# yaramohamadi/Pairwise_Sample_Optimization

Measured on AMD Instinct MI355X. Metric: PSO train-step imgs/sec (paired 1024² SDXL) at 1/2/4/8 MI355X, higher is better.
Workload: dtype bf16; 1 GPU; C2: SDXL-Turbo PSO train step, LoRA r=32 grads, 2 pairs/GPU/micro-step, gas 2, 2-step sampler (T=1); global_batch=4, seq_len=4096, resolution=1024, parallelism=dp1, launch=eager

## Files before the change

pairwise_sample_optimization_amd/csrc/attention.hip:

```cpp
#include "common.h"

#include <type_traits>

#define ATT_D 64
#define ATT_KT 64
#define ATT_THREADS 256

typedef __attribute__((address_space(3))) s16x4 lds_s16x4;

__device__ __forceinline__ int swz_row(int r, int c) { return r * ATT_D + ((c ^ (r & 7)) << 3); }
__device__ __forceinline__ int swz_tr(int r, int c) { return r * ATT_D + ((c ^ (((r >> 1) & 3) << 1)) << 3); }

__device__ __forceinline__ s16x4 tr_read(const bf16_t* img, int r0, int col0, int lane) {
  const int li = lane & 15;
  const int q = li >> 2, p = li & 3;
  const int row = r0 + q;
  const int col = col0 + 4 * p;
  const int off = swz_tr(row, col >> 3) + (col & 7);
  return __builtin_amdgcn_ds_read_tr16_b64_v4i16((lds_s16x4*)(img + off));
}

__device__ __forceinline__ s16x4 tr_read_asm(const bf16_t* img, int r0, int col0, int lane) {
  const int li = lane & 15;
  const int q = li >> 2, p = li & 3;
// ... 380 lines not shown
#pragma unroll
          for (int r = 0; r < 4; ++r)
            if (kbase + kj * 16 + 4 * g + r >= a.Sk) s[qi][kj][r] = -INFINITY;
    }
    float mx[QI];
    bool grow = false;
#pragma unroll
    for (int qi = 0; qi < QI; ++qi) {
      float m = vmax3(s[qi][0][0], s[qi][0][1], s[qi][0][2]);
      m = vmax3(m, s[qi][0][3], s[qi][1][0]);
      m = vmax3(m, s[qi][1][1], s[qi][1][2]);
      m = vmax3(m, s[qi][1][3], s[qi][2][0]);
      m = vmax3(m, s[qi][2][1], s[qi][2][2]);
      m = vmax3(m, s[qi][2][3], s[qi][3][0]);
      m = vmax3(m, s[qi][3][1], s[qi][3][2]);
      m = vmax2(m, s[qi][3][3]);
      mx[qi] = LG ? m : rowmax4_asm(m);
      grow |= mx[qi] > m_run[qi] + thr;
    }
    if (__any(grow)) {
#pragma unroll
      for (int qi = 0; qi < QI; ++qi) {
        const float m_new = fmaxf(m_run[qi], LG ? rowmax4_asm(mx[qi]) : mx[qi]);
        const float alpha = fast_exp2((m_run[qi] - m_new) * c2);
        lsum[qi] *= alpha;
#pragma unroll
        for (int dt = 0; dt < 4; ++dt) o[qi][dt] *= alpha;
        m_run[qi] = m_new;
      }
    }
#pragma unroll
    for (int qi = 0; qi < QI; ++qi) {
      const float mc = m_run[qi] * c2;
#pragma unroll
      for (int kj = 0; kj < 4; ++kj)
#pragma unroll
        for (int r = 0; r < 4; ++r) s[qi][kj][r] = fast_exp2(fmaf(s[qi][kj][r], c2, -mc));
    }
    lds_wait8(vr0);
    s16x4 vr1[8];
#pragma unroll
    for (int dt = 0; dt < 4; ++dt) {
      vr1[2 * dt] = tr_read_imm<VOFF + 2 * 2048>(vbase[dt]);
      vr1[2 * dt + 1] = tr_read_imm<VOFF + 3 * 2048>(vbase[dt]);
    }
#pragma unroll
    for (int ks = 0; ks < 2; ++ks) {
      if (ks == 1) lds_wait8(vr1);
      bf16x8 pf[QI];
#pragma unroll
      for (int qi = 0; qi < QI; ++qi) {
        pf[qi] = pack_p(s[qi][2 * ks], s[qi][2 * ks + 1]);
        lsum[qi] = mfma16x16x32(ones, pf[qi], lsum[qi]);
      }
#pragma unroll
      for (int dt = 0; dt < 4; ++dt) {
        const bf16x8 vf = ks == 0 ? cat_frag(vr0[2 * dt], vr0[2 * dt + 1]) : cat_frag(vr1[2 * dt], vr1[2 * dt + 1]);
#pragma unroll
        for (int qi = 0; qi < QI; ++qi) o[qi][dt] = mfma16x16x32(vf, pf[qi], o[qi][dt]);
      }
    }
  };
  for (int kt = 0; kt < nkt; kt += STG) {
    tile(ic<0>{}, kt);
    if (kt + 1 < nkt) tile(ic<1>{}, kt + 1);
    if (kt + 2 < nkt) tile(ic<2>{}, kt + 2);
  }

  bf16_t* O = a.o + b * a.so_b + h * ATT_D;
#pragma unroll
  for (int qi = 0; qi < QI; ++qi) {
    const float l = lsum[qi][0];
    const int qr = q0 + qi * 16 + c;
    if (qr >= a.Sq) continue;
    const float inv = 1.f / l;
#pragma unroll
    for (int dt = 0; dt < 4; ++dt) {
      const f32x4 v = o[qi][dt];
      *reinterpret_cast<uint2*>(O + (long)qr * a.ldo + dt * 16 + 4 * g) =
          make_uint2(pack2bf(v[0] * inv, v[1] * inv), pack2bf(v[2] * inv, v[3] * inv));
    }
    if (a.lse && g == 0)
      a.lse[((long)b * a.H + h) * a.Sq + qr] = (m_run[qi] * c2 + log2f(l)) * 0.69314718055994531f;
  }
}

template <int KJ, int STG, bool PF = false, bool ONE = false>
__global__ __launch_bounds__(ATT_THREADS, KJ == 2 ? 2 : 1) void attn_bwd_dkv_kernel(AttnArgs a, int nkb) {
  constexpr int IMG = ATT_KT * ATT_D;
  constexpr int NIMG = ONE ? 2 : 4;
  constexpr int PIECES = 2 * NIMG;
  extern __shared__ __attribute__((aligned(16))) bf16_t att_dyn[];
  bf16_t* const sbase = att_dyn;
  float* const sLD = reinterpret_cast<float*>(att_dyn + STG * NIMG * IMG);
  const int tid = threadIdx.x, lane = tid & 63;
  const int wave = __builtin_amdgcn_readfirstlane(tid >> 6);
  const int g = lane >> 4, c = lane & 15;
  const int bid = xcd_remap(blockIdx.x, gridDim.x);
  const int per_bh = nkb * a.q_split;
  const int bh = bid / per_bh, rem = bid - bh * per_bh;
  const int split = rem / nkb, kb = rem - split * nkb;
  const int h = bh % a.H, b = bh / a.H;
  const int k0 = kb * (64 * KJ) + wave * (16 * KJ);

  const bf16_t* Q = a.q + b * a.sq_b + h * ATT_D;
  const bf16_t* K = a.k + b * a.sk_b + h * ATT_D;
  const bf16_t* V = a.v + b * a.sv_b + h * ATT_D;
  const bf16_t* DO = a.dO + b * a.sdo_b + h * ATT_D;
  const float* LSE = a.lse2 + ((long)b * a.H + h) * a.Sq;
  const float* DEL = a.delta + ((long)b * a.H + h) * a.Sq;
  const float c2 = a.scale_log2;

  const int nqt = (a.Sq + ATT_KT - 1) / ATT_KT;
  const int per = (nqt + a.q_split - 1) / a.q_split;
  const int qa = split * per, qb = min(nqt, qa + per);
  const int n = qb > qa ? qb - qa : 0;

  const int prow = lane >> 3, pch = lane & 7;
  const int lcR = pch ^ prow;
  const int lcT = pch ^ (2 * ((prow >> 1) & 3));
  const __amdgpu_buffer_rsrc_t rQ =
      __builtin_amdgcn_make_buffer_rsrc((void*)Q, (short)0, (int)(((long)(a.Sq - 1) * a.ldq + ATT_D) * 2), 0x00020000);
  const __amdgpu_buffer_rsrc_t rO =
      __builtin_amdgcn_make_buffer_rsrc((void*)DO, (short)0, (int)(((long)(a.Sq - 1) * a.lddo + ATT_D) * 2), 0x00020000);
  const __amdgpu_buffer_rsrc_t rL =
      __builtin_amdgcn_make_buffer_rsrc((void*)(wave == 0 ? LSE : DEL), (short)0, a.Sq * 4, 0x00020000);
  unsigned qro[2], qto[2], oro[2], oto[2];
#pragma unroll
  for (int pw = 0; pw < 2; ++pw) {
    const int row = (wave * 2 + pw) * 8 + prow;
    qro[pw] = (unsigned)(row * (int)a.ldq + lcR * 8) * 2u;
    qto[pw] = (unsigned)(row * (int)a.ldq + lcT * 8) * 2u;
    oro[pw] = (unsigned)(row * (int)a.lddo + lcR * 8) * 2u;
    oto[pw] = (unsigned)(row * (int)a.lddo + lcT * 8) * 2u;
  }
  const int qstep = ATT_KT * (int)a.ldq * 2, ostep = ATT_KT * (int)a.lddo * 2;
  auto issue = [&](int qt, int buf) {
    bf16_t* img = sbase + buf * NIMG * IMG;
    if (wave < 2)
      __builtin_amdgcn_raw_ptr_buffer_load_lds(rL, (att_lds_void*)(sLD + (buf * 2 + wave) * 64), 4, lane * 4,
                                               qt * ATT_KT * 4, 0, 0);
#pragma unroll
    for (int pw = 0; pw < 2; ++pw) {
      const int piece = wave * 2 + pw;
      if constexpr (ONE) {
        __builtin_amdgcn_raw_ptr_buffer_load_lds(rQ, (att_lds_void*)(img + piece * 8 * ATT_D), 16, qto[pw], qt * qstep,
                                                 0, 0);
        __builtin_amdgcn_raw_ptr_buffer_load_lds(rO, (att_lds_void*)(img + IMG + piece * 8 * ATT_D), 16, oto[pw],
                                                 qt * ostep, 0, 0);
        continue;
      }
      __builtin_amdgcn_raw_ptr_buffer_load_lds(rQ, (att_lds_void*)(img + piece * 8 * ATT_D), 16, qro[pw], qt * qstep, 0, 0);
      __builtin_amdgcn_raw_ptr_buffer_load_lds(rQ, (att_lds_void*)(img + IMG + piece * 8 * ATT_D), 16, qto[pw], qt * qstep,
                                               0, 0);
      __builtin_amdgcn_raw_ptr_buffer_load_lds(rO, (att_lds_void*)(img + 2 * IMG + piece * 8 * ATT_D), 16, oro[pw],
                                               qt * ostep, 0, 0);
      __builtin_amdgcn_raw_ptr_buffer_load_lds(rO, (att_lds_void*)(img + 3 * IMG + piece * 8 * ATT_D), 16, oto[pw],
                                               qt * ostep, 0, 0);
    }
  };

  bf16x8 kf[KJ][2], vf[KJ][2];
#pragma unroll
  for (int kj = 0; kj < KJ; ++kj) {
    const int kr = min(k0 + kj * 16 + c, a.Sk - 1);
#pragma unroll
// ... 798 lines not shown
#pragma unroll
          for (int r = 0; r < 4; ++r) dsT[qi][kj][r] = fast_exp2(fmaf(sacc[r], a.scale_log2, -lq[qi])) * pacc[r];
        }
      }
    }
    s16x4 kr[2][8];
#pragma unroll
    for (int ks = 0; ks < 2; ++ks)
#pragma unroll
      for (int dt = 0; dt < 4; ++dt) {
        kr[ks][2 * dt] = tr_read_asm(sKt, (2 * ks) * 16 + 4 * g, dt * 16, lane);
        kr[ks][2 * dt + 1] = tr_read_asm(sKt, (2 * ks + 1) * 16 + 4 * g, dt * 16, lane);
      }
    bf16x8 pf[2][2];
#pragma unroll
    for (int ks = 0; ks < 2; ++ks)
#pragma unroll
      for (int qi = 0; qi < 2; ++qi) pf[ks][qi] = pack_p(dsT[qi][2 * ks], dsT[qi][2 * ks + 1]);
    lds_wait8(kr[0]);
    lds_wait8(kr[1]);
#pragma unroll
    for (int ks = 0; ks < 2; ++ks) {
#pragma unroll
      for (int dt = 0; dt < 4; ++dt) {
        const bf16x8 kf = cat_frag(kr[ks][2 * dt], kr[ks][2 * dt + 1]);
#pragma unroll
        for (int qi = 0; qi < 2; ++qi)
          dq[qi][dt] = mfma16x16x32(kf, pf[ks][qi], dq[qi][dt]);
      }
    }
    };
    if (kbase + ATT_KT > a.Sk) body(std::true_type{});
    else body(std::false_type{});
  };
  for (int kt = 0; kt < nkt; kt += STG) {
    tile(ic<0>{}, kt);
    if (kt + 1 < nkt) tile(ic<1>{}, kt + 1);
    if (kt + 2 < nkt) tile(ic<2>{}, kt + 2);
    if constexpr (STG > 3)
      if (kt + 3 < nkt) tile(ic<3>{}, kt + 3);
  }
  const float sc = a.scale_log2 * 0.69314718055994531f;
  bf16_t* DQ = a.dq + b * a.sdq_b + h * ATT_D;
#pragma unroll
  for (int qi = 0; qi < 2; ++qi) {
    const int qr = q0 + qi * 16 + c;
    if (qr >= a.Sq) continue;
#pragma unroll
    for (int dt = 0; dt < 4; ++dt) {
      const f32x4 v = dq[qi][dt];
      *reinterpret_cast<uint2*>(DQ + (long)qr * a.lddq + dt * 16 + 4 * g) =
          make_uint2(pack2bf(v[0] * sc, v[1] * sc), pack2bf(v[2] * sc, v[3] * sc));
    }
  }
}

__global__ void reduce_splits_kernel(long rows, int cols, int nsplit, const float* __restrict__ src_k,
                                     const float* __restrict__ src_v, long split_stride, bf16_t* __restrict__ dst_k,
                                     long ldd_k, bf16_t* __restrict__ dst_v, long ldd_v) {
  const float* __restrict__ src = blockIdx.y ? src_v : src_k;
  bf16_t* __restrict__ dst = blockIdx.y ? dst_v : dst_k;
  const long ldd = blockIdx.y ? ldd_v : ldd_k;
  const int c4 = cols / 4;
  for (long i = blockIdx.x * (long)blockDim.x + threadIdx.x; i < rows * c4; i += (long)gridDim.x * blockDim.x) {
    const long r = i / c4;
    const int cc = (int)(i - r * c4) * 4;
    float4 acc = *reinterpret_cast<const float4*>(src + r * cols + cc);
    for (int sp = 1; sp < nsplit; ++sp) {
      const float4 v = *reinterpret_cast<const float4*>(src + sp * split_stride + r * cols + cc);
      acc.x += v.x; acc.y += v.y; acc.z += v.z; acc.w += v.w;
    }
    *reinterpret_cast<uint2*>(dst + r * ldd + cc) = make_uint2(pack2bf(acc.x, acc.y), pack2bf(acc.z, acc.w));
  }
}

#ifdef PSO_BENCH_KNOBS
static int g_attn_fwd_variant = 0;
static bool g_attn_vsum = false;
static int g_attn_bwd_variant = 0;
static bool g_attn_pp_trace = false;
static int g_attn_xqs = 0;
#else
static constexpr int g_attn_fwd_variant = 0, g_attn_bwd_variant = 0, g_attn_xqs = 0;
#endif

static int cross_qsplit(int B, int H, int Sq, int Sk) {
  if (Sk > 256) return 1;
  if (Sk <= XK_KP && g_attn_bwd_variant != 7) {
    int qs = g_attn_xqs > 0 ? g_attn_xqs : 512 / (H * B);
    const int nqt = cdiv(Sq, ATT_KT);
    if (qs > nqt) qs = nqt;
    return qs < 1 ? 1 : qs;
  }
  const int nqt = cdiv(Sq, ATT_KT);
  int qs = cdiv(512, (long)cdiv(Sk, 128) * H * B);
  if (qs > nqt) qs = nqt;
  return qs < 1 ? 1 : qs;
}


static bool a16(const void* p, long ld) { return (((uintptr_t)p) & 15) == 0 && (ld % 8) == 0; }
static bool a8(const void* p, long ld) { return (((uintptr_t)p) & 7) == 0 && (ld % 4) == 0; }

extern "C" {

#ifdef PSO_BENCH_KNOBS
int pso_attn_pp_trace(unsigned long long* out) {
  return hipMemcpyFromSymbol(out, HIP_SYMBOL(g_pp_trace), sizeof(g_pp_trace)) == hipSuccess ? 0 : 1;
}

void pso_attention_set_variant(int v) {
  g_attn_fwd_variant = v % 10;
  g_attn_bwd_variant = (v / 10) % 10;
  g_attn_vsum = (v / 100) % 10 == 1;
  g_attn_pp_trace = (v / 1000) % 10 == 1;
  g_attn_xqs = (v / 10000) % 100;
}
#endif

int pso_attention_fwd(int B, int H, int Sq, int Sk, const void* q, long ldq, long sq_b, const void* k, long ldk,
                      long sk_b, const void* v, long ldv, long sv_b, float scale, void* o, long ldo, long so_b,
                      float* lse, void* stream) {
  PSO_ARG_CHECK(B > 0 && H > 0 && Sq > 0 && Sk > 0, "pso_attention_fwd: bad shape");
  PSO_ARG_CHECK(q && k && v && o, "pso_attention_fwd: null");
  PSO_ARG_CHECK(a16(q, ldq) && a16(k, ldk) && a16(v, ldv) && (((uintptr_t)o) & 7) == 0 && (ldo % 4) == 0,
                "pso_attention_fwd: operands need 16-B aligned rows");
  AttnArgs a{};
  a.q = (const bf16_t*)q; a.k = (const bf16_t*)k; a.v = (const bf16_t*)v;
  a.ldq = ldq; a.ldk = ldk; a.ldv = ldv; a.sq_b = sq_b; a.sk_b = sk_b; a.sv_b = sv_b;
  a.o = (bf16_t*)o; a.ldo = ldo; a.so_b = so_b; a.lse = lse;
  a.Sq = Sq; a.Sk = Sk; a.H = H; a.scale_log2 = scale * 1.4426950408889634f;
  const int nq4 = cdiv(Sq, 256), nq2 = cdiv(Sq, 128);
  const int fv = g_attn_fwd_variant;
  const int qsel = fv >= 5 ? fv - 5 : fv;
  const bool big = qsel == 4 || ((qsel == 0 || qsel == 1) && (long)nq4 * H * B >= 1024 && Sk > 128);
  hipStream_t st = (hipStream_t)stream;
#ifdef PSO_BENCH_KNOBS
  if (g_attn_vsum) {
    if (big) attn_fwd_kernel<4, false><<<nq4 * H * B, ATT_THREADS, 0, st>>>(a, nq4);
    else attn_fwd_kernel<2, false><<<nq2 * H * B, ATT_THREADS, 0, st>>>(a, nq2);
    return pso_check_launch("pso_attention_fwd");
  } else if (fv >= 5) {
    if (big) attn_fwd_kernel<4><<<nq4 * H * B, ATT_THREADS, 0, st>>>(a, nq4);
    else attn_fwd_kernel<2><<<nq2 * H * B, ATT_THREADS, 0, st>>>(a, nq2);
    return pso_check_launch("pso_attention_fwd");
  } else if (fv == 1) {
    if (big) attn_fwd2_kernel<4, true><<<nq4 * H * B, ATT_THREADS, 0, st>>>(a, nq4);
    else attn_fwd2_kernel<2, true><<<nq2 * H * B, ATT_THREADS, 0, st>>>(a, nq2);
    return pso_check_launch("pso_attention_fwd");
  }
#endif
  if (big) {
    attn_fwd2_kernel<4><<<nq4 * H * B, ATT_THREADS, 0, st>>>(a, nq4);
  } else {
    attn_fwd2_kernel<2><<<nq2 * H * B, ATT_THREADS, 0, st>>>(a, nq2);
  }
  return pso_check_launch("pso_attention_fwd");
}

size_t pso_attention_bwd_ws_bytes(int B, int H, int Sq, int Sk) {
  size_t d = (size_t)B * H * Sq * sizeof(float);
  const int qs = cross_qsplit(B, H, Sq, Sk);
  size_t acc = qs > 1 ? 2 * (size_t)qs * B * Sk * H * ATT_D * sizeof(float) : 0;
  return 2 * (((d + 255) / 256) * 256) + acc;
}

int pso_attention_bwd(int B, int H, int Sq, int Sk, const void* q, long ldq, long sq_b, const void* k, long ldk,
                      long sk_b, const void* v, long ldv, long sv_b, const void* o, long ldo, long so_b,
                      const float* lse, const void* dO, long lddo, long sdo_b, float scale, void* dq, long lddq,
                      long sdq_b, void* dk, long lddk, long sdk_b, void* dv, long lddv, long sdv_b, void* ws,
                      size_t ws_bytes, void* stream) {
  PSO_ARG_CHECK(B > 0 && H > 0 && Sq > 0 && Sk > 0, "pso_attention_bwd: bad shape");
  PSO_ARG_CHECK(q && k && v && o && lse && dO && dq && dk && dv && ws, "pso_attention_bwd: null");
  PSO_ARG_CHECK(ws_bytes >= pso_attention_bwd_ws_bytes(B, H, Sq, Sk), "pso_attention_bwd: workspace too small");
  PSO_ARG_CHECK(a16(q, ldq) && a16(k, ldk) && a16(v, ldv) && a16(o, ldo) && a16(dO, lddo),
                "pso_attention_bwd: operands need 16-B aligned rows");
  PSO_ARG_CHECK(a8(dq, lddq) && a8(dk, lddk) && a8(dv, lddv),
                "pso_attention_bwd: dq/dk/dv need 8-B aligned rows (pointer % 8 == 0, row stride % 4 == 0)");
  PSO_ARG_CHECK(cross_qsplit(B, H, Sq, Sk) == 1 || (sdk_b == (long)Sk * lddk && sdv_b == (long)Sk * lddv),
                "pso_attention_bwd: the query-split path needs dk/dv batch strides of Sk rows "
                "(sdk_b == Sk*lddk, sdv_b == Sk*lddv)");
  hipStream_t st = (hipStream_t)stream;
  AttnArgs a{};
  a.q = (const bf16_t*)q; a.k = (const bf16_t*)k; a.v = (const bf16_t*)v;
  a.ldq = ldq; a.ldk = ldk; a.ldv = ldv; a.sq_b = sq_b; a.sk_b = sk_b; a.sv_b = sv_b;
  a.o = (bf16_t*)o; a.ldo = ldo; a.so_b = so_b; a.lse = (float*)lse;
  a.Sq = Sq; a.Sk = Sk; a.H = H; a.scale_log2 = scale * 1.4426950408889634f;
  a.dO = (const bf16_t*)dO; a.lddo = lddo; a.sdo_b = sdo_b;
  const size_t dsz = (((size_t)B * H * Sq * sizeof(float) + 255) / 256) * 256;
  float* delta = (float*)ws;
  a.delta = delta;
  a.lse2 = (float*)((char*)ws + dsz);
  a.dq = (bf16_t*)dq; a.dk = (bf16_t*)dk; a.dv = (bf16_t*)dv;
  a.lddq = lddq; a.lddk = lddk; a.lddv = lddv; a.sdq_b = sdq_b; a.sdk_b = sdk_b; a.sdv_b = sdv_b;
  const size_t doff = 2 * dsz;
  const int nkb = cdiv(Sk, 128);
  const int qsplit = cross_qsplit(B, H, Sq, Sk);
  const long part = (long)B * Sk * H * ATT_D;
  if (qsplit > 1) {
    a.dk_acc = (float*)((char*)ws + doff);
    a.dv_acc = a.dk_acc + qsplit * part;
  }
  a.q_split = qsplit;
  a.nbatch = B;
  const dim3 gq(cdiv(Sq, 128), H, B);
  const bool xpath = Sk <= XK_KP && g_attn_bwd_variant != 7;
  if (xpath) {
    attn_bwd_x_kernel<<<dim3(qsplit * H * B), ATT_THREADS, 0, st>>>(a);
  } else {
#ifdef PSO_BENCH_KNOBS
  const int bv = g_attn_bwd_variant;
  if (bv == 3 || bv == 1) attn_bwd_dq_kernel<3, false><<<gq, ATT_THREADS, 0, st>>>(a);
  else if (bv == 6) attn_bwd_dq_kernel<4, true><<<gq, ATT_THREADS, 0, st>>>(a);
  else attn_bwd_dq_kernel<3, true><<<gq, ATT_THREADS, 0, st>>>(a);
  const int nkb4 = cdiv(Sk, 256);
  const bool kj4 = g_attn_bwd_variant == 4;
  if (kj4) {
    const size_t shm = 3 * (4 * ATT_KT * ATT_D * sizeof(bf16_t) + 2 * 64 * sizeof(float));
    static bool attr4 = false;
    if (!attr4) {
      (void)hipFuncSetAttribute((const void*)attn_bwd_dkv_kernel<4, 3>, hipFuncAttributeMaxDynamicSharedMemorySize,
                                (int)shm);
      attr4 = true;
    }
    attn_bwd_dkv_kernel<4, 3><<<nkb4 * qsplit * H * B, ATT_THREADS, shm, st>>>(a, nkb4);
  } else if ((bv == 8 || bv == 9) && qsplit == 1) {
    constexpr int PST = 4;
    const size_t shm = PST * (2 * ATT_KT * ATT_D * sizeof(bf16_t) + 2 * 64 * sizeof(float));
    static bool attr8 = false;
    if (!attr8) {
      (void)hipFuncSetAttribute((const void*)attn_bwd_dkv_pp_kernel<PST>, hipFuncAttributeMaxDynamicSharedMemorySize,
                                (int)shm);
      (void)hipFuncSetAttribute((const void*)attn_bwd_dkv_pp_kernel<PST, true>,
                                hipFuncAttributeMaxDynamicSharedMemorySize, (int)shm);
// ... 50 lines not shown
```

pairwise_sample_optimization_amd/csrc/gemm_skinny.hip:

```cpp
#include "common.h"

#include <cstdlib>

__device__ __attribute__((aligned(16))) uint4 g_skinny_zero[4];

namespace {

constexpr int SK_W = 8;

template <int NJ, int SK_MT, int SK_U_ = 0>
__global__ __launch_bounds__(64 * SK_W) void gemm_skinny_nt_kernel(int M, int N, int K, const bf16_t* __restrict__ A,
                                                                   long lda, const bf16_t* __restrict__ W, long ldw,
                                                                   float alpha, void* __restrict__ out, long ldo,
                                                                   int out_f32, int accumulate) {
  constexpr int SK_U = SK_U_ > 0 ? SK_U_ : ((NJ <= 2 && SK_MT <= 2) ? 4 : 2);
  __shared__ f32x4 red[SK_W][NJ][64];
  const int lane = threadIdx.x & 63, wave = threadIdx.x >> 6;
  const int fr = lane & 15, fk = lane >> 4;
  const int r0 = blockIdx.x * (16 * SK_MT);
  const int grp = blockIdx.y;
  A += (long)grp * K;
  W += (long)grp * K;
  const bf16_t* zero = reinterpret_cast<const bf16_t*>(g_skinny_zero);
  const bf16_t* arow[SK_MT];
#pragma unroll
  for (int t = 0; t < SK_MT; ++t) arow[t] = A + (long)min(r0 + t * 16 + fr, M - 1) * lda;
  const bf16_t* wrow[NJ];
  bool wok[NJ];
#pragma unroll
  for (int j = 0; j < NJ; ++j) {
    wok[j] = j * 16 + fr < N;
    wrow[j] = W + (long)min(j * 16 + fr, N - 1) * ldw;
  }
  const int nc = (K + 31) / 32;
  f32x4 acc[SK_MT][NJ];
#pragma unroll
  for (int t = 0; t < SK_MT; ++t)
#pragma unroll
    for (int j = 0; j < NJ; ++j) acc[t][j] = f32x4{0.f, 0.f, 0.f, 0.f};

  for (int c0 = wave; c0 < nc; c0 += SK_W * SK_U) {
    bf16x8 af[SK_U][SK_MT], bfr[SK_U][NJ];
#pragma unroll
    for (int u = 0; u < SK_U; ++u) {
      const int k = (c0 + u * SK_W) * 32 + fk * 8;
      const bool ok = k < K;
#pragma unroll
      for (int t = 0; t < SK_MT; ++t) af[u][t] = *reinterpret_cast<const bf16x8*>(ok ? arow[t] + k : zero);
#pragma unroll
      for (int j = 0; j < NJ; ++j) bfr[u][j] = *reinterpret_cast<const bf16x8*>((ok && wok[j]) ? wrow[j] + k : zero);
    }
    __builtin_amdgcn_sched_barrier(0);
#pragma unroll
    for (int u = 0; u < SK_U; ++u)
#pragma unroll
      for (int t = 0; t < SK_MT; ++t)
#pragma unroll
        for (int j = 0; j < NJ; ++j)
          acc[t][j] = mfma16x16x32(bfr[u][j], af[u][t], acc[t][j]);
  }
#pragma unroll
  for (int t = 0; t < SK_MT; ++t) {
    if (t > 0) __syncthreads();
#pragma unroll
    for (int j = 0; j < NJ; ++j) red[wave][j][lane] = acc[t][j];
    __syncthreads();
    for (int idx = threadIdx.x; idx < NJ * 64; idx += 64 * SK_W) {
      const int l = idx & 63, j = idx >> 6;
      f32x4 s = red[0][j][l];
#pragma unroll
      for (int w = 1; w < SK_W; ++w) s += red[w][j][l];
      const int m = r0 + t * 16 + (l & 15);
      const int n = j * 16 + (l >> 4) * 4;
      if (m >= M || n >= N) continue;
      float v0 = s[0] * alpha, v1 = s[1] * alpha, v2 = s[2] * alpha, v3 = s[3] * alpha;
      const long o = (long)m * ldo + (long)grp * N + n;
      if (out_f32) {
        float4* po = reinterpret_cast<float4*>(reinterpret_cast<float*>(out) + o);
        if (accumulate) {
          const float4 old = *po;
          v0 += old.x; v1 += old.y; v2 += old.z; v3 += old.w;
        }
        *po = make_float4(v0, v1, v2, v3);
      } else {
        *reinterpret_cast<uint2*>(reinterpret_cast<bf16_t*>(out) + o) = make_uint2(pack2bf(v0, v1), pack2bf(v2, v3));
      }
    }
  }
}

#ifdef PSO_BENCH_KNOBS
static int skinny_variant() {
  static int v = -1;
  if (v < 0) {
    const char* e = getenv("PSO_SKINNY_VARIANT");
    v = e ? atoi(e) : 0;
  }
  return v;
}
#else
static constexpr int skinny_variant() { return 0; }
#endif

template <int NJ>
int launch_skinny(int M, int N, int K, const bf16_t* a, long lda, const bf16_t* w, long ldw, float alpha, void* out,
                  long ldo, int out_f32, int accumulate, int groups, hipStream_t st) {
  const int var = NJ <= 2 ? skinny_variant() : 0;
#ifdef PSO_BENCH_KNOBS
  if (var == 1 || var == 3) {
    const dim3 grid((M + 15) / 16, groups);
    if (var == 1) {
      pso_note_kernel("gemm_skinny_nt_kernel<%d, %d, %d>", NJ, 1, 8);
      gemm_skinny_nt_kernel<NJ, 1, 8><<<grid, 64 * SK_W, 0, st>>>(M, N, K, a, lda, w, ldw, alpha, out, ldo, out_f32,
                                                                    accumulate);
    } else {
      pso_note_kernel("gemm_skinny_nt_kernel<%d, %d, %d>", NJ, 1, 4);
      gemm_skinny_nt_kernel<NJ, 1, 4><<<grid, 64 * SK_W, 0, st>>>(M, N, K, a, lda, w, ldw, alpha, out, ldo, out_f32,
                                                                    accumulate);
    }
    return pso_check_launch("pso_gemm(skinny)");
  }
  if (var == 2) {
    const dim3 grid((M + 31) / 32, groups);
    pso_note_kernel("gemm_skinny_nt_kernel<%d, %d, %d>", NJ, 2, 8);
    gemm_skinny_nt_kernel<NJ, 2, 8><<<grid, 64 * SK_W, 0, st>>>(M, N, K, a, lda, w, ldw, alpha, out, ldo, out_f32,
                                                                accumulate);
    return pso_check_launch("pso_gemm(skinny)");
  }
#endif
  const bool k40 = var != 4 && (K + 31) / 32 > SK_W * 4 && (K + 31) / 32 <= SK_W * 5;
  const bool five = NJ <= 6 && k40, five4 = NJ <= 2 && k40;
  constexpr int U5 = NJ <= 6 ? 5 : 4, U5m = NJ <= 6 ? 5 : 0, U5d = NJ <= 2 ? 5 : 0;
  if ((long)((M + 31) / 32) * groups < 128) {
    const dim3 grid((M + 15) / 16, groups);
    if (five) {
      pso_note_kernel("gemm_skinny_nt_kernel<%d, %d, %d>", NJ, 1, U5);
      gemm_skinny_nt_kernel<NJ, 1, U5><<<grid, 64 * SK_W, 0, st>>>(M, N, K, a, lda, w, ldw, alpha, out, ldo, out_f32,
                                                                    accumulate);
    } else {
      pso_note_kernel("gemm_skinny_nt_kernel<%d, %d, %d>", NJ, 1, 4);
      gemm_skinny_nt_kernel<NJ, 1, 4><<<grid, 64 * SK_W, 0, st>>>(M, N, K, a, lda, w, ldw, alpha, out, ldo, out_f32,
                                                                    accumulate);
    }
  } else if ((long)((M + 63) / 64) * groups >= 256) {
    const dim3 grid((M + 63) / 64, groups);
    if (five4) {
      pso_note_kernel("gemm_skinny_nt_kernel<%d, %d, %d>", NJ, 4, U5d);
      gemm_skinny_nt_kernel<NJ, 4, U5d><<<grid, 64 * SK_W, 0, st>>>(M, N, K, a, lda, w, ldw, alpha, out, ldo, out_f32,
                                                                    accumulate);
    } else {
      pso_note_kernel("gemm_skinny_nt_kernel<%d, %d, 0>", NJ, 4);
      gemm_skinny_nt_kernel<NJ, 4><<<grid, 64 * SK_W, 0, st>>>(M, N, K, a, lda, w, ldw, alpha, out, ldo, out_f32,
                                                               accumulate);
    }
  } else {
    const dim3 grid((M + 31) / 32, groups);
    if (five) {
      pso_note_kernel("gemm_skinny_nt_kernel<%d, %d, %d>", NJ, 2, U5m);
      gemm_skinny_nt_kernel<NJ, 2, U5m><<<grid, 64 * SK_W, 0, st>>>(M, N, K, a, lda, w, ldw, alpha, out, ldo, out_f32,
                                                                    accumulate);
    } else {
      pso_note_kernel("gemm_skinny_nt_kernel<%d, %d, 0>", NJ, 2);
      gemm_skinny_nt_kernel<NJ, 2><<<grid, 64 * SK_W, 0, st>>>(M, N, K, a, lda, w, ldw, alpha, out, ldo, out_f32,
                                                               accumulate);
    }
  }
  return pso_check_launch("pso_gemm(skinny)");
}

}

int pso_gemm_skinny_nt(int M, int N, int K, const void* A, long lda, const void* W, long ldw, float alpha, void* out,
                       long ldo, int out_f32, int accumulate, int groups, hipStream_t st) {
  const int nj = (N + 15) / 16;
  auto a = (const bf16_t*)A;
  auto w = (const bf16_t*)W;
  switch (nj) {
    case 1: return launch_skinny<1>(M, N, K, a, lda, w, ldw, alpha, out, ldo, out_f32, accumulate, groups, st);
    case 2: return launch_skinny<2>(M, N, K, a, lda, w, ldw, alpha, out, ldo, out_f32, accumulate, groups, st);
    case 3: case 4: return launch_skinny<4>(M, N, K, a, lda, w, ldw, alpha, out, ldo, out_f32, accumulate, groups, st);
    case 5: case 6: return launch_skinny<6>(M, N, K, a, lda, w, ldw, alpha, out, ldo, out_f32, accumulate, groups, st);
    default: return launch_skinny<8>(M, N, K, a, lda, w, ldw, alpha, out, ldo, out_f32, accumulate, groups, st);
  }
}
```

Before: 37.99 imgs/s.

## Add dedicated cross-attention forward kernel and coalesced row loads in skinny GEMM

Adds attn_fwd_x_kernel for short-key (cross) attention. It keeps the whole K/V (at most two tiles) resident in LDS and loops several query blocks per workgroup, with a q-split grid. Output rows are staged through per-wave LDS so stores are coalesced 16-byte rows. Separately, the skinny GEMM now loads A/W as contiguous row lines and transposes the fragments across lanes with ds_bpermute, trading extra cross-lane permutes for better global-load coalescing. Both paths are on by default, and the old skinny layout is only reachable through a bench knob.

```diff
diff --git a/pairwise_sample_optimization_amd/csrc/attention.hip b/pairwise_sample_optimization_amd/csrc/attention.hip
--- a/pairwise_sample_optimization_amd/csrc/attention.hip
+++ b/pairwise_sample_optimization_amd/csrc/attention.hip
@@ -486,6 +486,242 @@
     }
     if (a.lse && g == 0)
       a.lse[((long)b * a.H + h) * a.Sq + qr] = (m_run[qi] * c2 + log2f(l)) * 0.69314718055994531f;
+  }
+}
+
+__global__ __launch_bounds__(ATT_THREADS, 3) void attn_fwd_x_kernel(AttnArgs a, int nqb, int qsplit) {
+  constexpr int QI = 2;
+  constexpr int OLD = ATT_D + 8;
+  __shared__ __attribute__((aligned(16))) bf16_t sKV[2][2][ATT_KT * ATT_D];
+  __shared__ __attribute__((aligned(16))) bf16_t sO[ATT_THREADS / 64][16 * OLD];
+  const int tid = threadIdx.x, lane = tid & 63;
+  const int wave = __builtin_amdgcn_readfirstlane(tid >> 6);
+  const int g = lane >> 4, c = lane & 15;
+  const int lr = lane >> 2, lc = lane & 3;
+  const int bid = xcd_remap(blockIdx.x, gridDim.x);
+  const int bh = bid / qsplit, split = bid - bh * qsplit;
+  const int h = bh % a.H, b = bh / a.H;
+  const int per = (nqb + qsplit - 1) / qsplit;
+  const int qa = split * per, qe = min(nqb, qa + per);
+  if (qa >= qe) return;
+
+  const bf16_t* Q = a.q + b * a.sq_b + h * ATT_D;
+  const bf16_t* K = a.k + b * a.sk_b + h * ATT_D;
+  const bf16_t* V = a.v + b * a.sv_b + h * ATT_D;
+  bf16_t* O = a.o + b * a.so_b + h * ATT_D;
+  const float c2 = a.scale_log2;
+  const float thr = ATT_RESCALE_LOG2 / c2;
+
+  auto qload = [&](uint4 (&r)[QI][2], int qb) {
+#pragma unroll
+    for (int qi = 0; qi < QI; ++qi) {
+      const int qr = min(qb * (64 * QI) + wave * (16 * QI) + qi * 16 + lr, a.Sq - 1);
+#pragma unroll
+      for (int ds = 0; ds < 2; ++ds)
+        r[qi][ds] = *reinterpret_cast<const uint4*>(Q + (long)qr * a.ldq + ds * 32 + 8 * lc);
+    }
+  };
+  uint4 qraw[QI][2];
+  qload(qraw, qa);
+
+  const int prow = lane >> 3, pch = lane & 7;
+  const int lcK = pch ^ prow;
+  const int lcV = pch ^ (2 * ((prow >> 1) & 3));
+  const int nkt = (a.Sk + ATT_KT - 1) / ATT_KT;
+  const __amdgpu_buffer_rsrc_t rK =
+      __builtin_amdgcn_make_buffer_rsrc((void*)K, (short)0, (int)(((long)(a.Sk - 1) * a.ldk + ATT_D) * 2), 0x00020000);
+  const __amdgpu_buffer_rsrc_t rV =
+      __builtin_amdgcn_make_buffer_rsrc((void*)V, (short)0, (int)(((long)(a.Sk - 1) * a.ldv + ATT_D) * 2), 0x00020000);
+  const int kstep = ATT_KT * (int)a.ldk * 2, vstep = ATT_KT * (int)a.ldv * 2;
+#pragma unroll
+  for (int kt = 0; kt < 2; ++kt) {
+    if (kt < nkt) {
+#pragma unroll
+      for (int pw = 0; pw < 2; ++pw) {
+        const int piece = wave * 2 + pw;
+        const int row = piece * 8 + prow;
+        __builtin_amdgcn_raw_ptr_buffer_load_lds(rK, (att_lds_void*)(sKV[kt][0] + piece * 8 * ATT_D), 16,
+                                                 (unsigned)(row * (int)a.ldk + lcK * 8) * 2u, kt * kstep, 0, 0);
+        __builtin_amdgcn_raw_ptr_buffer_load_lds(rV, (att_lds_void*)(sKV[kt][1] + piece * 8 * ATT_D), 16,
+                                                 (unsigned)(row * (int)a.ldv + lcV * 8) * 2u, kt * vstep, 0, 0);
+      }
+    }
+  }
+  unsigned vbase[4];
+  {
+    const unsigned lds0 = (unsigned)(uintptr_t)(const att_lds_void*)&sKV[0][0][0];
+    const int li = lane & 15, q = li >> 2, p = li & 3;
+#pragma unroll
+    for (int dt = 0; dt < 4; ++dt) {
+      const int col = dt * 16 + 4 * p;
+      vbase[dt] = lds0 + 2u * (unsigned)(swz_tr(4 * g + q, col >> 3) + (col & 7));
+    }
+  }
+  asm volatile("s_waitcnt vmcnt(0)\n\ts_barrier" ::: "memory");
+
+  const bf16x8 ones = __builtin_bit_cast(bf16x8, make_uint4(PSO_ELEM_ONES2, PSO_ELEM_ONES2, PSO_ELEM_ONES2, PSO_ELEM_ONES2));
+  const int xsrc = (4 * c + g) * 4;
+  bf16_t* so = sO[wave];
+
+  for (int qb = qa; qb < qe; ++qb) {
+    const int q0 = qb * (64 * QI) + wave * (16 * QI);
+    bf16x8 qf[QI][2];
+#pragma unroll
+    for (int qi = 0; qi < QI; ++qi)
+#pragma unroll
+      for (int ds = 0; ds < 2; ++ds) {
+        uint4 x = qraw[qi][ds];
+        x.x = __builtin_amdgcn_ds_bpermute(xsrc, x.x);
+        x.y = __builtin_amdgcn_ds_bpermute(xsrc, x.y);
+        x.z = __builtin_amdgcn_ds_bpermute(xsrc, x.z);
+        x.w = __builtin_amdgcn_ds_bpermute(xsrc, x.w);
+        qf[qi][ds] = __builtin_bit_cast(bf16x8, x);
+      }
+    if (qb + 1 < qe) qload(qraw, qb + 1);
+
+    f32x4 o[QI][4];
+    f32x4 lsum[QI];
+    float m_run[QI];
+#pragma unroll
+    for (int qi = 0; qi < QI; ++qi) {
+      m_run[qi] = -INFINITY;
+      lsum[qi] = f32x4{0.f, 0.f, 0.f, 0.f};
+#pragma unroll
+      for (int dt = 0; dt < 4; ++dt) o[qi][dt] = f32x4{0.f, 0.f, 0.f, 0.f};
+    }
+    auto tile = [&](auto bufc, int kt) {
+      constexpr int buf = decltype(bufc)::value;
+      const bf16_t* k_img = sKV[buf][0];
+      const int nl = min(4, (a.Sk - kt * ATT_KT + 15) >> 4);
+      f32x4 s[QI][4];
+#pragma unroll
+      for (int kj = 0; kj < 4; ++kj) {
+        if (kj >= nl) {
+#pragma unroll
+          for (int qi = 0; qi < QI; ++qi) s[qi][kj] = f32x4{-INFINITY, -INFINITY, -INFINITY, -INFINITY};
+          continue;
+        }
+        bf16x8 kf[2];
+#pragma unroll
+        for (int ds = 0; ds < 2; ++ds)
+          kf[ds] = *reinterpret_cast<const bf16x8*>(k_img + swz_row(kj * 16 + c, ds * 4 + g));
+#pragma unroll
+        for (int qi = 0; qi < QI; ++qi) {
+          f32x4 acc = {0.f, 0.f, 0.f, 0.f};
+          acc = mfma16x16x32(kf[0], qf[qi][0], acc);
+          s[qi][kj] = mfma16x16x32(kf[1], qf[qi][1], acc);
+        }
+      }
+      constexpr int VOFF = (buf * 2 + 1) * ATT_KT * ATT_D * 2;
+      s16x4 vr0[8];
+#pragma unroll
+      for (int dt = 0; dt < 4; ++dt) {
+        vr0[2 * dt] = tr_read_imm<VOFF + 0 * 2048>(vbase[dt]);
+        vr0[2 * dt + 1] = tr_read_imm<VOFF + 1 * 2048>(vbase[dt]);
+      }
+      const int kbase = kt * ATT_KT;
+      if (kbase + ATT_KT > a.Sk) {
+#pragma unroll
+        for (int qi = 0; qi < QI; ++qi)
+#pragma unroll
+          for (int kj = 0; kj < 4; ++kj)
+#pragma unroll
+            for (int r = 0; r < 4; ++r)
+              if (kbase + kj * 16 + 4 * g + r >= a.Sk) s[qi][kj][r] = -INFINITY;
+      }
+      float mx[QI];
+      bool grow = false;
+#pragma unroll
+      for (int qi = 0; qi < QI; ++qi) {
+        float m = vmax3(s[qi][0][0], s[qi][0][1], s[qi][0][2]);
+        m = vmax3(m, s[qi][0][3], s[qi][1][0]);
+        m = vmax3(m, s[qi][1][1], s[qi][1][2]);
+        m = vmax3(m, s[qi][1][3], s[qi][2][0]);
+        m = vmax3(m, s[qi][2][1], s[qi][2][2]);
+        m = vmax3(m, s[qi][2][3], s[qi][3][0]);
+        m = vmax3(m, s[qi][3][1], s[qi][3][2]);
+        m = vmax2(m, s[qi][3][3]);
+        mx[qi] = rowmax4_asm(m);
+        grow |= mx[qi] > m_run[qi] + thr;
+      }
+      if (__any(grow)) {
+#pragma unroll
+        for (int qi = 0; qi < QI; ++qi) {
+          const float m_new = fmaxf(m_run[qi], mx[qi]);
+          const float alpha = fast_exp2((m_run[qi] - m_new) * c2);
+          lsum[qi] *= alpha;
+#pragma unroll
+          for (int dt = 0; dt < 4; ++dt) o[qi][dt] *= alpha;
+          m_run[qi] = m_new;
+        }
+      }
+#pragma unroll
+      for (int qi = 0; qi < QI; ++qi) {
+        const float mc = m_run[qi] * c2;
+#pragma unroll
+        for (int kj = 0; kj < 4; ++kj) {
+          if (kj < nl) {
+#pragma unroll
+            for (int r = 0; r < 4; ++r) s[qi][kj][r] = fast_exp2(fmaf(s[qi][kj][r], c2, -mc));
+          } else {
+            s[qi][kj] = f32x4{0.f, 0.f, 0.f, 0.f};
+          }
+        }
+      }
+      lds_wait8(vr0);
+      s16x4 vr1[8];
+      if (nl > 2) {
+#pragma unroll
+        for (int dt = 0; dt < 4; ++dt) {
+          vr1[2 * dt] = tr_read_imm<VOFF + 2 * 2048>(vbase[dt]);
+          vr1[2 * dt + 1] = tr_read_imm<VOFF + 3 * 2048>(vbase[dt]);
+        }
+      }
+#pragma unroll
+      for (int ks = 0; ks < 2; ++ks) {
+        if (2 * ks >= nl) continue;
+        if (ks == 1) lds_wait8(vr1);
+        bf16x8 pf[QI];
+#pragma unroll
+        for (int qi = 0; qi < QI; ++qi) {
+          pf[qi] = pack_p(s[qi][2 * ks], s[qi][2 * ks + 1]);
+          lsum[qi] = mfma16x16x32(ones, pf[qi], lsum[qi]);
+        }
+#pragma unroll
+        for (int dt = 0; dt < 4; ++dt) {
+          const bf16x8 vf = ks == 0 ? cat_frag(vr0[2 * dt], vr0[2 * dt + 1]) : cat_frag(vr1[2 * dt], vr1[2 * dt + 1]);
+#pragma unroll
+          for (int qi = 0; qi < QI; ++qi) o[qi][dt] = mfma16x16x32(vf, pf[qi], o[qi][dt]);
+        }
+      }
+    };
+    tile(ic<0>{}, 0);
+    if (nkt > 1) tile(ic<1>{}, 1);
+
+#pragma unroll
+    for (int qi = 0; qi < QI; ++qi) {
+      const float l = lsum[qi][0];
+      const float inv = 1.f / l;
+      asm volatile("" ::: "memory");
+      __builtin_amdgcn_wave_barrier();
+#pragma unroll
+      for (int dt = 0; dt < 4; ++dt) {
+        const f32x4 v = o[qi][dt];
+        *reinterpret_cast<uint2*>(so + c * OLD + dt * 16 + 4 * g) =
+            make_uint2(pack2bf(v[0] * inv, v[1] * inv), pack2bf(v[2] * inv, v[3] * inv));
+      }
+      asm volatile("" ::: "memory");
+      __builtin_amdgcn_wave_barrier();
+      const int orow = q0 + qi * 16 + lr;
+#pragma unroll
+      for (int sx = 0; sx < 2; ++sx) {
+        const uint4 w = *reinterpret_cast<const uint4*>(so + lr * OLD + (lc + 4 * sx) * 8);
+        if (orow < a.Sq) *reinterpret_cast<uint4*>(O + (long)orow * a.ldo + (lc + 4 * sx) * 8) = w;
+      }
+      const int qr = q0 + qi * 16 + c;
+      if (a.lse && g == 0 && qr < a.Sq)
+        a.lse[((long)b * a.H + h) * a.Sq + qr] = (m_run[qi] * c2 + log2f(l)) * 0.69314718055994531f;
+    }
   }
 }
 
@@ -1450,6 +1686,7 @@
 static int g_attn_xqs = 0;
 #else
 static constexpr int g_attn_fwd_variant = 0, g_attn_bwd_variant = 0, g_attn_xqs = 0;
+static constexpr bool g_attn_vsum = false;
 #endif
 
 static int cross_qsplit(int B, int H, int Sq, int Sk) {
@@ -1500,9 +1737,17 @@
   a.Sq = Sq; a.Sk = Sk; a.H = H; a.scale_log2 = scale * 1.4426950408889634f;
   const int nq4 = cdiv(Sq, 256), nq2 = cdiv(Sq, 128);
   const int fv = g_attn_fwd_variant;
-  const int qsel = fv >= 5 ? fv - 5 : fv;
+  const int qsel = fv >= 5 ? fv - 5 : (fv == 3 ? 0 : fv);
   const bool big = qsel == 4 || ((qsel == 0 || qsel == 1) && (long)nq4 * H * B >= 1024 && Sk > 128);
   hipStream_t st = (hipStream_t)stream;
+  if (Sk <= XK_KP && fv == 0 && !g_attn_vsum && a16(o, ldo) && so_b % 8 == 0) {
+    int qs = 768 / (H * B);
+    if (qs > nq2) qs = nq2;
+    if (qs < 1) qs = 1;
+    pso_note_kernel("attn_fwd_x_kernel");
+    attn_fwd_x_kernel<<<B * H * qs, ATT_THREADS, 0, st>>>(a, nq2, qs);
+    return pso_check_launch("pso_attention_fwd");
+  }
 #ifdef PSO_BENCH_KNOBS
   if (g_attn_vsum) {
     if (big) attn_fwd_kernel<4, false><<<nq4 * H * B, ATT_THREADS, 0, st>>>(a, nq4);
@@ -1518,6 +1763,7 @@
     return pso_check_launch("pso_attention_fwd");
   }
 #endif
+  pso_note_kernel("attn_fwd2_kernel<%d, false>", big ? 4 : 2);
   if (big) {
     attn_fwd2_kernel<4><<<nq4 * H * B, ATT_THREADS, 0, st>>>(a, nq4);
   } else {
diff --git a/pairwise_sample_optimization_amd/csrc/gemm_skinny.hip b/pairwise_sample_optimization_amd/csrc/gemm_skinny.hip
--- a/pairwise_sample_optimization_amd/csrc/gemm_skinny.hip
+++ b/pairwise_sample_optimization_amd/csrc/gemm_skinny.hip
@@ -8,7 +8,15 @@
 
 constexpr int SK_W = 8;
 
-template <int NJ, int SK_MT, int SK_U_ = 0>
+__device__ __forceinline__ bf16x8 lane_xpose(bf16x8 v, int src) {
+  typedef __attribute__((ext_vector_type(4))) int i32x4;
+  i32x4 x = __builtin_bit_cast(i32x4, v);
+#pragma unroll
+  for (int d = 0; d < 4; ++d) x[d] = __builtin_amdgcn_ds_bpermute(src, x[d]);
+  return __builtin_bit_cast(bf16x8, x);
+}
+
+template <int NJ, int SK_MT, int SK_U_ = 0, bool LINE = true>
 __global__ __launch_bounds__(64 * SK_W) void gemm_skinny_nt_kernel(int M, int N, int K, const bf16_t* __restrict__ A,
                                                                    long lda, const bf16_t* __restrict__ W, long ldw,
                                                                    float alpha, void* __restrict__ out, long ldo,
@@ -17,6 +25,8 @@
   __shared__ f32x4 red[SK_W][NJ][64];
   const int lane = threadIdx.x & 63, wave = threadIdx.x >> 6;
   const int fr = lane & 15, fk = lane >> 4;
+  const int lr = LINE ? lane >> 2 : fr, lk = LINE ? lane & 3 : fk;
+  const int xsrc = (4 * fr + fk) * 4;
   const int r0 = blockIdx.x * (16 * SK_MT);
   const int grp = blockIdx.y;
   A += (long)grp * K;
@@ -24,13 +34,13 @@
   const bf16_t* zero = reinterpret_cast<const bf16_t*>(g_skinny_zero);
   const bf16_t* arow[SK_MT];
 #pragma unroll
-  for (int t = 0; t < SK_MT; ++t) arow[t] = A + (long)min(r0 + t * 16 + fr, M - 1) * lda;
+  for (int t = 0; t < SK_MT; ++t) arow[t] = A + (long)min(r0 + t * 16 + lr, M - 1) * lda;
   const bf16_t* wrow[NJ];
   bool wok[NJ];
 #pragma unroll
   for (int j = 0; j < NJ; ++j) {
-    wok[j] = j * 16 + fr < N;
-    wrow[j] = W + (long)min(j * 16 + fr, N - 1) * ldw;
+    wok[j] = j * 16 + lr < N;
+    wrow[j] = W + (long)min(j * 16 + lr, N - 1) * ldw;
   }
   const int nc = (K + 31) / 32;
   f32x4 acc[SK_MT][NJ];
@@ -43,7 +53,7 @@
     bf16x8 af[SK_U][SK_MT], bfr[SK_U][NJ];
 #pragma unroll
     for (int u = 0; u < SK_U; ++u) {
-      const int k = (c0 + u * SK_W) * 32 + fk * 8;
+      const int k = (c0 + u * SK_W) * 32 + lk * 8;
       const bool ok = k < K;
 #pragma unroll
       for (int t = 0; t < SK_MT; ++t) af[u][t] = *reinterpret_cast<const bf16x8*>(ok ? arow[t] + k : zero);
@@ -52,12 +62,19 @@
     }
     __builtin_amdgcn_sched_barrier(0);
 #pragma unroll
-    for (int u = 0; u < SK_U; ++u)
+    for (int u = 0; u < SK_U; ++u) {
+      if (LINE) {
+#pragma unroll
+        for (int j = 0; j < NJ; ++j) bfr[u][j] = lane_xpose(bfr[u][j], xsrc);
+#pragma unroll
+        for (int t = 0; t < SK_MT; ++t) af[u][t] = lane_xpose(af[u][t], xsrc);
+      }
 #pragma unroll
       for (int t = 0; t < SK_MT; ++t)
 #pragma unroll
         for (int j = 0; j < NJ; ++j)
           acc[t][j] = mfma16x16x32(bfr[u][j], af[u][t], acc[t][j]);
+    }
   }
 #pragma unroll
   for (int t = 0; t < SK_MT; ++t) {
@@ -91,16 +108,56 @@
 
 #ifdef PSO_BENCH_KNOBS
 static int skinny_variant() {
-  static int v = -1;
-  if (v < 0) {
-    const char* e = getenv("PSO_SKINNY_VARIANT");
-    v = e ? atoi(e) : 0;
-  }
-  return v;
+  const char* e = getenv("PSO_SKINNY_VARIANT");
+  return e ? atoi(e) : 0;
 }
 #else
 static constexpr int skinny_variant() { return 0; }
 #endif
+
+template <int NJ, bool LINE>
+int launch_skinny_auto(int var, int M, int N, int K, const bf16_t* a, long lda, const bf16_t* w, long ldw, float alpha,
+                       void* out, long ldo, int out_f32, int accumulate, int groups, hipStream_t st) {
+  const bool k40 = var != 4 && (K + 31) / 32 > SK_W * 4 && (K + 31) / 32 <= SK_W * 5;
+  const bool five = NJ <= 6 && k40, five4 = NJ <= 2 && k40;
+  constexpr int U5 = NJ <= 6 ? 5 : 4, U5m = NJ <= 6 ? 5 : 0, U5d = NJ <= 2 ? 5 : 0;
+  if ((long)((M + 31) / 32) * groups < 128) {
+    const dim3 grid((M + 15) / 16, groups);
+    if (five) {
+      pso_note_kernel("gemm_skinny_nt_kernel<%d, %d, %d>", NJ, 1, U5);
+      gemm_skinny_nt_kernel<NJ, 1, U5, LINE><<<grid, 64 * SK_W, 0, st>>>(M, N, K, a, lda, w, ldw, alpha, out, ldo, out_f32,
+                                                                    accumulate);
+    } else {
+      pso_note_kernel("gemm_skinny_nt_kernel<%d, %d, %d>", NJ, 1, 4);
+      gemm_skinny_nt_kernel<NJ, 1, 4, LINE><<<grid, 64 * SK_W, 0, st>>>(M, N, K, a, lda, w, ldw, alpha, out, ldo,
+                                                                          out_f32, accumulate);
+    }
+  } else if ((long)((M + 63) / 64) * groups >= 256) {
+    const dim3 grid((M + 63) / 64, groups);
+    if (five4) {
+      pso_note_kernel("gemm_skinny_nt_kernel<%d, %d, %d>", NJ, 4, U5d);
+      gemm_skinny_nt_kernel<NJ, 4, U5d, LINE><<<grid, 64 * SK_W, 0, st>>>(M, N, K, a, lda, w, ldw, alpha, out, ldo, out_f32,
+                                                                    accumulate);
+    } else {
+      pso_note_kernel("gemm_skinny_nt_kernel<%d, %d, 0>", NJ, 4);
+      gemm_skinny_nt_kernel<NJ, 4, 0, LINE><<<grid, 64 * SK_W, 0, st>>>(M, N, K, a, lda, w, ldw, alpha, out, ldo, out_f32,
+                                                               accumulate);
+    }
+  } else {
+    const dim3 grid((M + 31) / 32, groups);
+    if (five) {
+      pso_note_kernel("gemm_skinny_nt_kernel<%d, %d, %d>", NJ, 2, U5m);
+      gemm_skinny_nt_kernel<NJ, 2, U5m, LINE><<<grid, 64 * SK_W, 0, st>>>(M, N, K, a, lda, w, ldw, alpha, out, ldo, out_f32,
+                                                                    accumulate);
+    } else {
+      pso_note_kernel("gemm_skinny_nt_kernel<%d, %d, 0>", NJ, 2);
+      gemm_skinny_nt_kernel<NJ, 2, 0, LINE><<<grid, 64 * SK_W, 0, st>>>(M, N, K, a, lda, w, ldw, alpha, out, ldo, out_f32,
+                                                               accumulate);
+    }
+  }
+  return pso_check_launch("pso_gemm(skinny)");
+}
+
 
 template <int NJ>
 int launch_skinny(int M, int N, int K, const bf16_t* a, long lda, const bf16_t* w, long ldw, float alpha, void* out,
@@ -111,61 +168,26 @@
     const dim3 grid((M + 15) / 16, groups);
     if (var == 1) {
       pso_note_kernel("gemm_skinny_nt_kernel<%d, %d, %d>", NJ, 1, 8);
-      gemm_skinny_nt_kernel<NJ, 1, 8><<<grid, 64 * SK_W, 0, st>>>(M, N, K, a, lda, w, ldw, alpha, out, ldo, out_f32,
+      gemm_skinny_nt_kernel<NJ, 1, 8, false><<<grid, 64 * SK_W, 0, st>>>(M, N, K, a, lda, w, ldw, alpha, out, ldo, out_f32,
                                                                     accumulate);
     } else {
       pso_note_kernel("gemm_skinny_nt_kernel<%d, %d, %d>", NJ, 1, 4);
-      gemm_skinny_nt_kernel<NJ, 1, 4><<<grid, 64 * SK_W, 0, st>>>(M, N, K, a, lda, w, ldw, alpha, out, ldo, out_f32,
-                                                                    accumulate);
+      gemm_skinny_nt_kernel<NJ, 1, 4, false><<<grid, 64 * SK_W, 0, st>>>(M, N, K, a, lda, w, ldw, alpha, out, ldo,
+                                                                           out_f32, accumulate);
     }
     return pso_check_launch("pso_gemm(skinny)");
   }
   if (var == 2) {
     const dim3 grid((M + 31) / 32, groups);
     pso_note_kernel("gemm_skinny_nt_kernel<%d, %d, %d>", NJ, 2, 8);
-    gemm_skinny_nt_kernel<NJ, 2, 8><<<grid, 64 * SK_W, 0, st>>>(M, N, K, a, lda, w, ldw, alpha, out, ldo, out_f32,
+    gemm_skinny_nt_kernel<NJ, 2, 8, false><<<grid, 64 * SK_W, 0, st>>>(M, N, K, a, lda, w, ldw, alpha, out, ldo, out_f32,
                                                                 accumulate);
     return pso_check_launch("pso_gemm(skinny)");
   }
+  if (skinny_variant() == 5)
+    return launch_skinny_auto<NJ, false>(0, M, N, K, a, lda, w, ldw, alpha, out, ldo, out_f32, accumulate, groups, st);
 #endif
-  const bool k40 = var != 4 && (K + 31) / 32 > SK_W * 4 && (K + 31) / 32 <= SK_W * 5;
-  const bool five = NJ <= 6 && k40, five4 = NJ <= 2 && k40;
-  constexpr int U5 = NJ <= 6 ? 5 : 4, U5m = NJ <= 6 ? 5 : 0, U5d = NJ <= 2 ? 5 : 0;
-  if ((long)((M + 31) / 32) * groups < 128) {
-    const dim3 grid((M + 15) / 16, groups);
-    if (five) {
-      pso_note_kernel("gemm_skinny_nt_kernel<%d, %d, %d>", NJ, 1, U5);
-      gemm_skinny_nt_kernel<NJ, 1, U5><<<grid, 64 * SK_W, 0, st>>>(M, N, K, a, lda, w, ldw, alpha, out, ldo, out_f32,
-                                                                    accumulate);
-    } else {
-      pso_note_kernel("gemm_skinny_nt_kernel<%d, %d, %d>", NJ, 1, 4);
-      gemm_skinny_nt_kernel<NJ, 1, 4><<<grid, 64 * SK_W, 0, st>>>(M, N, K, a, lda, w, ldw, alpha, out, ldo, out_f32,
-                                                                    accumulate);
-    }
-  } else if ((long)((M + 63) / 64) * groups >= 256) {
-    const dim3 grid((M + 63) / 64, groups);
-    if (five4) {
-      pso_note_kernel("gemm_skinny_nt_kernel<%d, %d, %d>", NJ, 4, U5d);
-      gemm_skinny_nt_kernel<NJ, 4, U5d><<<grid, 64 * SK_W, 0, st>>>(M, N, K, a, lda, w, ldw, alpha, out, ldo, out_f32,
-                                                                    accumulate);
-    } else {
-      pso_note_kernel("gemm_skinny_nt_kernel<%d, %d, 0>", NJ, 4);
-      gemm_skinny_nt_kernel<NJ, 4><<<grid, 64 * SK_W, 0, st>>>(M, N, K, a, lda, w, ldw, alpha, out, ldo, out_f32,
-                                                               accumulate);
-    }
-  } else {
-    const dim3 grid((M + 31) / 32, groups);
-    if (five) {
-      pso_note_kernel("gemm_skinny_nt_kernel<%d, %d, %d>", NJ, 2, U5m);
-      gemm_skinny_nt_kernel<NJ, 2, U5m><<<grid, 64 * SK_W, 0, st>>>(M, N, K, a, lda, w, ldw, alpha, out, ldo, out_f32,
-                                                                    accumulate);
-    } else {
-      pso_note_kernel("gemm_skinny_nt_kernel<%d, %d, 0>", NJ, 2);
-      gemm_skinny_nt_kernel<NJ, 2><<<grid, 64 * SK_W, 0, st>>>(M, N, K, a, lda, w, ldw, alpha, out, ldo, out_f32,
-                                                               accumulate);
-    }
-  }
-  return pso_check_launch("pso_gemm(skinny)");
+  return launch_skinny_auto<NJ, true>(var, M, N, K, a, lda, w, ldw, alpha, out, ldo, out_f32, accumulate, groups, st);
 }
 
 }
```

Result: no change. 38.12 imgs/s (median of 6 runs) (+0.4%).
